# alibaba/EasyParallelLibrary

Measured on AMD Instinct MI355X. Metric: samples_per_sec, higher is better.
Workload: dtype bf16; 1 GPU; model=bert-large, global_batch=128, seq_len=512, parallelism=dp1

## Files before the change

csrc/bindings.hip:

```cpp

#include <hip/hip_runtime.h>
#include <torch/extension.h>
#include <ATen/hip/impl/HIPStreamMasqueradingAsCUDA.h>

#include <cstdint>

namespace epl {
void register_comm(py::module& m);
}

extern "C" {
void epl_fused_adamw(float*, unsigned short*, const void*, bool, float*,
                     float*, int64_t, float, float, float, float, float, int,
                     float, hipStream_t);
void epl_lamb_phase1(const float*, const void*, bool, float*, float*, float*,
                     const int*, float*, float*, int64_t, float, float, float,
                     float, int, float, hipStream_t);
void epl_lamb_phase2(float*, unsigned short*, const float*, const int*,
                     const float*, int64_t, float, hipStream_t);
void epl_layer_norm_fwd(void*, const void*, const void*, void*, const void*,
                        const void*, float*, float*, int64_t, int64_t, float,
                        bool, hipStream_t);
void epl_layer_norm_bwd(void*, float*, float*, const void*, const void*,
                        const void*, const float*, const float*, float*,
                        float*, int64_t, int64_t, int64_t, bool,
                        hipStream_t);
void epl_bias_gelu_fwd(void*, const void*, const void*, int64_t, int64_t,
                       bool, hipStream_t);
void epl_bias_gelu_bwd(void*, float*, const void*, const void*, const void*,
                       float*, int64_t, int64_t, int64_t, bool,
                       hipStream_t);
void epl_ce_rowstats(const void*, const int64_t*, float*, float*, float*,
                     int64_t, int64_t, int64_t, int64_t, bool, hipStream_t);
void epl_ce_backward(void*, const void*, const int64_t*, const float*,
                     const float*, const float*, int64_t, int64_t, int64_t,
                     int64_t, float, bool, hipStream_t);
void epl_scale(void*, int64_t, float, bool, hipStream_t);
void epl_f32_to_bf16(unsigned short*, const float*, int64_t, hipStream_t);
void epl_bf16_to_f32(float*, const unsigned short*, int64_t, hipStream_t);
void epl_sqnorm(const void*, int64_t, float*, bool, hipStream_t);
void epl_colsum(void*, const void*, float*, int64_t, int64_t, int64_t,
                bool, hipStream_t);
void run_mfma_probe(const unsigned short*, const unsigned short*, float*,
                    hipStream_t);
void run_tr_read_probe(short*, short*, int, hipStream_t);
void epl_moe_dispatch_fwd(void*, const void*, const int64_t*,
                          const int64_t*, const int64_t*, int64_t, int64_t,
                          int64_t, hipStream_t);
void epl_moe_dispatch_bwd(void*, const void*, const int64_t*,
                          const int64_t*, const int64_t*, int64_t, int64_t,
                          int64_t, int64_t, hipStream_t);
void epl_moe_combine_fwd(void*, const void*, const float*, const int64_t*,
                         const int64_t*, const int64_t*, int64_t, int64_t,
                         int64_t, int64_t, hipStream_t);
void epl_moe_combine_bwd(void*, float*, const void*, const void*,
                         const float*, const int64_t*, const int64_t*,
                         const int64_t*, int64_t, int64_t, int64_t,
                         hipStream_t);
void epl_attn_fwd(const void*, const void*, const void*, void*, float*,
// ... 107 lines not shown
                     cols, (float)eps, bf16, cur_stream());
}

void layer_norm_bwd(at::Tensor dx, at::Tensor dgamma, at::Tensor dbeta,
                    at::Tensor dy, at::Tensor x, at::Tensor gamma,
                    at::Tensor mean, at::Tensor rstd) {
  const bool bf16 = is_bf16(x);
  const int64_t cols = x.size(-1);
  const int64_t rows = x.numel() / cols;
  TORCH_CHECK(!bf16 || cols % 8 == 0, "bf16 LayerNorm needs cols % 8 == 0");
  TORCH_CHECK((size_t)cols * 2 * sizeof(float) <= 128 * 1024,
              "LayerNorm backward supports cols <= 16384");
  check(dgamma, at::kFloat, "dgamma");
  check(dbeta, at::kFloat, "dbeta");
  float* dgp = nullptr;
  float* dbp = nullptr;
  at::Tensor ws;
  const bool fast = bf16 && cols % 8 == 0 && cols <= 2048;
  int64_t nparts = 0;
  if (fast) {
    const int64_t wave_rows = (rows + 3) / 4;
    nparts = (wave_rows < 1024 ? wave_rows : 1024) * 4;
    ws = at::empty({2, nparts, cols}, dgamma.options());
    dgp = ws.data_ptr<float>();
    dbp = dgp + nparts * cols;
  }
  epl_layer_norm_bwd(dx.data_ptr(), dgamma.data_ptr<float>(),
                     dbeta.data_ptr<float>(), dy.data_ptr(), x.data_ptr(),
                     gamma.data_ptr(), mean.data_ptr<float>(),
                     rstd.data_ptr<float>(), dgp, dbp, nparts, rows, cols,
                     bf16, cur_stream());
}

void bias_gelu_fwd(at::Tensor out, at::Tensor x, at::Tensor bias) {
  const bool bf16 = is_bf16(x);
  const int64_t cols = x.size(-1);
  const int64_t rows = x.numel() / cols;
  TORCH_CHECK(!bf16 || cols % 8 == 0, "bf16 bias_gelu needs cols % 8 == 0");
  epl_bias_gelu_fwd(out.data_ptr(), x.data_ptr(), bias.data_ptr(), rows, cols,
                    bf16, cur_stream());
}

void bias_gelu_bwd(at::Tensor dx, at::Tensor dbias, at::Tensor dy,
                   at::Tensor x, at::Tensor bias) {
  const bool bf16 = is_bf16(x);
  const int64_t cols = x.size(-1);
  const int64_t rows = x.numel() / cols;
  TORCH_CHECK(!bf16 || cols % 8 == 0, "bf16 bias_gelu needs cols % 8 == 0");
  TORCH_CHECK((size_t)cols * sizeof(float) <= 128 * 1024,
              "bias_gelu backward supports cols <= 32768");
  check(dbias, at::kFloat, "dbias");
  float* dbp = nullptr;
  int64_t nwaves = 0;
  at::Tensor ws;
  if (bf16 && cols % 512 == 0) {
    const int64_t segs = cols / 512;
    int64_t per_seg = rows < 1024 ? rows : 1024;
    per_seg = (per_seg + 3) / 4 * 4;
    nwaves = segs * per_seg;
    ws = at::empty({nwaves, 512}, dbias.options());
    dbp = ws.data_ptr<float>();
  }
  epl_bias_gelu_bwd(dx.data_ptr(), dbias.data_ptr<float>(), dy.data_ptr(),
                    x.data_ptr(), bias.data_ptr(), dbp, nwaves, rows, cols,
                    bf16, cur_stream());
}
// ... 220 lines not shown
}

void colsum(at::Tensor dy, at::Tensor db, at::Tensor partial) {
  const bool bf16 = is_bf16(dy);
  TORCH_CHECK(dy.is_cuda() && dy.is_contiguous() && dy.dim() == 2,
              "dy must be a contiguous 2-D device tensor");
  const int64_t rows = dy.size(0), cols = dy.size(1);
  TORCH_CHECK(cols % 8 == 0, "cols must be a multiple of 8");
  TORCH_CHECK(db.numel() == cols && db.scalar_type() == dy.scalar_type());
  const int64_t stripes = partial.numel() / cols;
  TORCH_CHECK(stripes >= 1 && partial.scalar_type() == at::kFloat);
  epl_colsum(db.data_ptr(), dy.data_ptr(), partial.data_ptr<float>(), rows,
             cols, stripes, bf16, cur_stream());
}

void sqnorm(at::Tensor t, at::Tensor out) {
  const bool bf16 = is_bf16(t);
  check(out, at::kFloat, "out");
  epl_sqnorm(t.data_ptr(), t.numel(), out.data_ptr<float>(), bf16,
             cur_stream());
}

}

PYBIND11_MODULE(TORCH_EXTENSION_NAME, m) {
  m.doc() = "MI355X-native parallel library: RCCL comm core + CDNA4 kernels";
  epl::register_comm(m);
  m.def("fused_adamw", &fused_adamw);
  m.def("colsum", &colsum);
  m.def("lamb_phase1", &lamb_phase1);
  m.def("lamb_phase2", &lamb_phase2);
  m.def("layer_norm_fwd", &layer_norm_fwd);
  m.def("layer_norm_bwd", &layer_norm_bwd);
  m.def("bias_gelu_fwd", &bias_gelu_fwd);
  m.def("bias_gelu_bwd", &bias_gelu_bwd);
  m.def("ce_rowstats", &ce_rowstats);
  m.def("ce_backward", &ce_backward);
  m.def("scale_", &scale_);
  m.def("f32_to_bf16", &f32_to_bf16);
  m.def("bf16_to_f32", &bf16_to_f32);
  m.def("sqnorm", &sqnorm);
  m.def("mfma_probe", &mfma_probe);
  m.def("tr_read_probe", &tr_read_probe);
  m.def("moe_dispatch_fwd", &moe_dispatch_fwd);
  m.def("moe_dispatch_bwd", &moe_dispatch_bwd);
  m.def("moe_combine_fwd", &moe_combine_fwd);
  m.def("moe_combine_bwd", &moe_combine_bwd);
  m.def("attn_fwd", &attn_fwd);
  m.def("attn_bwd", &attn_bwd);
}
```

csrc/kernels/kernels.hip:

```cpp

#include <hip/hip_runtime.h>
#include <hip/hip_bf16.h>
#include <cstdint>
#include <cmath>

#define DEV __device__ __forceinline__

namespace {

constexpr int kBlock = 256;
constexpr int kMaxGrid = 4096;

DEV float bf2f(unsigned short u) {
  unsigned int x = (unsigned int)u << 16;
  return __uint_as_float(x);
}

DEV unsigned short f2bf(float f) {
  unsigned int x = __float_as_uint(f);
  unsigned int lsb = (x >> 16) & 1u;
  x += 0x7fffu + lsb;
  return (unsigned short)(x >> 16);
}

// ... 266 lines not shown
          reinterpret_cast<float*>(sum_out)[base + c] = fv;
      }
      sum += fv;
      sumsq += fv * fv;
    }
    sum = block_reduce_sum(sum, lds);
    __syncthreads();
    sumsq = block_reduce_sum(sumsq, lds);
    const float mean = sum / cols;
    const float var = sumsq / cols - mean * mean;
    const float rstd = rsqrtf(var + eps);
    if (threadIdx.x == 0) {
      mean_out[row] = mean;
      rstd_out[row] = rstd;
    }
    const void* nin = HAS_RES ? sum_out : x;
    for (int64_t c = threadIdx.x; c < cols; c += blockDim.x) {
      float fv = BF16 ? bf2f(reinterpret_cast<const T*>(nin)[base + c])
                      : reinterpret_cast<const float*>(nin)[base + c];
      float gv = BF16 ? bf2f(reinterpret_cast<const T*>(gamma)[c])
                      : reinterpret_cast<const float*>(gamma)[c];
      float bv = BF16 ? bf2f(reinterpret_cast<const T*>(beta)[c])
                      : reinterpret_cast<const float*>(beta)[c];
      float y = (fv - mean) * rstd * gv + bv;
      if (BF16)
        reinterpret_cast<T*>(out)[base + c] = f2bf(y);
      else
        reinterpret_cast<float*>(out)[base + c] = y;
    }
    __syncthreads();
  }
}

template <int CHUNKS, bool CACHE>
__global__ __launch_bounds__(256, 2) void layer_norm_bwd_bf16_kernel(
    void* __restrict__ dx, float* __restrict__ dg_part,
    float* __restrict__ db_part, const void* __restrict__ dy,
    const void* __restrict__ x, const void* __restrict__ gamma,
    const float* __restrict__ mean_in, const float* __restrict__ rstd_in,
    int64_t rows, int64_t cols) {
  using T = unsigned short;
  const int lane = threadIdx.x & 63;
  const int wid = threadIdx.x >> 6;
  const int wpb = blockDim.x >> 6;
  float8 gw[CHUNKS], acc_dg[CHUNKS], acc_db[CHUNKS];
#pragma unroll
  for (int k = 0; k < CHUNKS; ++k) {
    const int64_t c = ((int64_t)lane + k * 64) * 8;
#pragma unroll
    for (int j = 0; j < 8; ++j) {
      acc_dg[k].v[j] = 0.f;
      acc_db[k].v[j] = 0.f;
    }
    if (c < cols)
      gw[k] = load_bf16x8(reinterpret_cast<const T*>(gamma) + c);
  }
  for (int64_t row = (int64_t)blockIdx.x * wpb + wid; row < rows;
       row += (int64_t)gridDim.x * wpb) {
    const int64_t base = row * cols;
    const float mean = mean_in[row];
    const float rstd = rstd_in[row];
    float sum_dyg = 0.f, sum_dygx = 0.f;
    float8 c_xhat[CACHE ? CHUNKS : 1], c_dy[CACHE ? CHUNKS : 1];
#pragma unroll
    for (int k = 0; k < CHUNKS; ++k) {
      const int64_t c = ((int64_t)lane + k * 64) * 8;
      if (c >= cols) continue;
      float8 d = load_bf16x8(reinterpret_cast<const T*>(dy) + base + c);
      float8 f = load_bf16x8(reinterpret_cast<const T*>(x) + base + c);
#pragma unroll
      for (int j = 0; j < 8; ++j) {
        const float xhat = (f.v[j] - mean) * rstd;
        const float dyg = d.v[j] * gw[k].v[j];
        if (CACHE) {
          c_xhat[k].v[j] = xhat;
          c_dy[k].v[j] = d.v[j];
        }
        sum_dyg += dyg;
        sum_dygx += dyg * xhat;
      }
    }
#pragma unroll
    for (int off = 32; off > 0; off >>= 1) {
      sum_dyg += __shfl_down(sum_dyg, off, 64);
      sum_dygx += __shfl_down(sum_dygx, off, 64);
    }
    sum_dyg = __shfl(sum_dyg, 0, 64);
    sum_dygx = __shfl(sum_dygx, 0, 64);
    const float inv_cols = 1.f / cols;
#pragma unroll
    for (int k = 0; k < CHUNKS; ++k) {
      const int64_t c = ((int64_t)lane + k * 64) * 8;
      if (c >= cols) continue;
      float8 dv, xh;
      if (CACHE) {
        dv = c_dy[k];
        xh = c_xhat[k];
      } else {
        float8 d = load_bf16x8(reinterpret_cast<const T*>(dy) + base + c);
        float8 f = load_bf16x8(reinterpret_cast<const T*>(x) + base + c);
#pragma unroll
        for (int j = 0; j < 8; ++j) {
          dv.v[j] = d.v[j];
          xh.v[j] = (f.v[j] - mean) * rstd;
        }
      }
      float8 o;
#pragma unroll
      for (int j = 0; j < 8; ++j) {
        const float dyg = dv.v[j] * gw[k].v[j];
        o.v[j] = (dyg - (sum_dyg + xh.v[j] * sum_dygx) * inv_cols) * rstd;
        acc_dg[k].v[j] += dv.v[j] * xh.v[j];
        acc_db[k].v[j] += dv.v[j];
      }
      store_bf16x8(reinterpret_cast<T*>(dx) + base + c, o);
    }
  }
  const int64_t prow = ((int64_t)blockIdx.x * wpb + wid) * cols;
#pragma unroll
  for (int k = 0; k < CHUNKS; ++k) {
    const int64_t c = ((int64_t)lane + k * 64) * 8;
    if (c >= cols) continue;
    store_f32x8(dg_part + prow + c, acc_dg[k]);
    store_f32x8(db_part + prow + c, acc_db[k]);
  }
}

__global__ void ln_bwd_partial_reduce_kernel(
    float* __restrict__ dgamma, float* __restrict__ dbeta,
    const float* __restrict__ dg_part, const float* __restrict__ db_part,
    int64_t nparts, int64_t cols) {
  const int64_t c = (int64_t)blockIdx.x * blockDim.x + threadIdx.x;
  if (c >= cols) return;
  float sg = 0.f, sb = 0.f;
  for (int64_t p = blockIdx.y; p < nparts; p += gridDim.y) {
    sg += dg_part[p * cols + c];
    sb += db_part[p * cols + c];
  }
  atomicAdd(&dgamma[c], sg);
  atomicAdd(&dbeta[c], sb);
}

template <bool BF16>
__global__ void layer_norm_bwd_kernel(
    void* __restrict__ dx, float* __restrict__ dgamma,
    float* __restrict__ dbeta, const void* __restrict__ dy,
    const void* __restrict__ x, const void* __restrict__ gamma,
    const float* __restrict__ mean_in, const float* __restrict__ rstd_in,
    int64_t rows, int64_t cols) {
  extern __shared__ __attribute__((aligned(16))) char smem[];
  float* part_dg = reinterpret_cast<float*>(smem);
  float* part_db = part_dg + cols;
  __shared__ float lds[8];
  using T = unsigned short;
  for (int64_t c = threadIdx.x; c < cols; c += blockDim.x) {
    part_dg[c] = 0.f;
    part_db[c] = 0.f;
  }
  __syncthreads();
  for (int64_t row = blockIdx.x; row < rows; row += gridDim.x) {
    const int64_t base = row * cols;
    const float mean = mean_in[row];
    const float rstd = rstd_in[row];
    float sum_dyg = 0.f, sum_dygx = 0.f;
    for (int64_t c = threadIdx.x; c < cols; c += blockDim.x) {
      const float dv = BF16 ? bf2f(reinterpret_cast<const T*>(dy)[base + c])
                            : reinterpret_cast<const float*>(dy)[base + c];
      const float fv = BF16 ? bf2f(reinterpret_cast<const T*>(x)[base + c])
                            : reinterpret_cast<const float*>(x)[base + c];
      const float gv = BF16 ? bf2f(reinterpret_cast<const T*>(gamma)[c])
                            : reinterpret_cast<const float*>(gamma)[c];
      const float xhat = (fv - mean) * rstd;
      const float dyg = dv * gv;
// ... 18 lines not shown
      const float o = (dv * gv - (sum_dyg + xhat * sum_dygx) * inv_cols) *
                      rstd;
      if (BF16)
        reinterpret_cast<T*>(dx)[base + c] = f2bf(o);
      else
        reinterpret_cast<float*>(dx)[base + c] = o;
    }
    __syncthreads();
  }
  for (int64_t c = threadIdx.x; c < cols; c += blockDim.x) {
    atomicAdd(&dgamma[c], part_dg[c]);
    atomicAdd(&dbeta[c], part_db[c]);
  }
}

DEV float fast_tanh(float u) {
  return 1.f - 2.f / (__expf(2.f * u) + 1.f);
}

DEV float gelu_f(float x) {
  const float k0 = 0.7978845608028654f;
  const float k1 = 0.044715f;
  return 0.5f * x * (1.f + fast_tanh(k0 * (x + k1 * x * x * x)));
}

DEV float gelu_grad_f(float x) {
  const float k0 = 0.7978845608028654f;
  const float k1 = 0.044715f;
  const float t = fast_tanh(k0 * (x + k1 * x * x * x));
  const float dt = (1.f - t * t) * k0 * (1.f + 3.f * k1 * x * x);
  return 0.5f * (1.f + t) + 0.5f * x * dt;
}

template <bool BF16>
__global__ void bias_gelu_fwd_kernel(void* __restrict__ out,
                                     const void* __restrict__ x,
                                     const void* __restrict__ bias,
                                     int64_t rows, int64_t cols) {
  using T = unsigned short;
  const int64_t n = rows * cols;
  if (BF16) {
    const int64_t nvec = n / 8;
    for (int64_t i = blockIdx.x * blockDim.x + threadIdx.x; i < nvec;
         i += (int64_t)gridDim.x * blockDim.x) {
      const int64_t base = i * 8;
      float8 f = load_bf16x8(reinterpret_cast<const T*>(x) + base);
      float8 b = load_bf16x8(reinterpret_cast<const T*>(bias) +
                             (base % cols));
      float8 o;
#pragma unroll
      for (int k = 0; k < 8; ++k) o.v[k] = gelu_f(f.v[k] + b.v[k]);
      store_bf16x8(reinterpret_cast<T*>(out) + base, o);
    }
  } else {
    for (int64_t i = blockIdx.x * blockDim.x + threadIdx.x; i < n;
         i += (int64_t)gridDim.x * blockDim.x) {
      const float xv = reinterpret_cast<const float*>(x)[i] +
                       reinterpret_cast<const float*>(bias)[i % cols];
      reinterpret_cast<float*>(out)[i] = gelu_f(xv);
    }
  }
}

__global__ void bias_gelu_bwd_bf16_kernel(
    void* __restrict__ dx, float* __restrict__ db_part,
    const void* __restrict__ dy, const void* __restrict__ x,
    const void* __restrict__ bias, int64_t rows, int64_t cols) {
  using T = unsigned short;
  const int lane = threadIdx.x & 63;
  const int wid = threadIdx.x >> 6;
  const int wpb = blockDim.x >> 6;
  const int64_t segs = cols / 512;
  const int64_t total = rows * segs;
  float8 acc;
#pragma unroll
  for (int j = 0; j < 8; ++j) acc.v[j] = 0.f;
  const int64_t wave_id = (int64_t)blockIdx.x * wpb + wid;
  const int64_t nwaves = (int64_t)gridDim.x * wpb;
  const int64_t myseg = wave_id % segs;
  const int64_t c0 = myseg * 512 + (int64_t)lane * 8;
  float8 bw = load_bf16x8(reinterpret_cast<const T*>(bias) + c0);
  for (int64_t row = wave_id / segs; row < rows; row += nwaves / segs) {
    const int64_t base = row * cols + c0;
    float8 d = load_bf16x8(reinterpret_cast<const T*>(dy) + base);
    float8 f = load_bf16x8(reinterpret_cast<const T*>(x) + base);
    float8 o;
#pragma unroll
    for (int j = 0; j < 8; ++j) {
      const float g = d.v[j] * gelu_grad_f(f.v[j] + bw.v[j]);
      o.v[j] = g;
      acc.v[j] += g;
    }
    store_bf16x8(reinterpret_cast<T*>(dx) + base, o);
  }
  store_f32x8(db_part + wave_id * 512 + (int64_t)lane * 8, acc);
}

__global__ void bias_gelu_db_reduce_kernel(
    float* __restrict__ dbias, const float* __restrict__ db_part,
    int64_t nwaves, int64_t segs) {
  const int64_t c = (int64_t)blockIdx.x * blockDim.x + threadIdx.x;
  if (c >= segs * 512) return;
  const int64_t seg = c / 512;
  const int64_t off = c % 512;
  float sum = 0.f;
  for (int64_t p = seg + blockIdx.y * segs; p < nwaves;
       p += (int64_t)gridDim.y * segs) {
    sum += db_part[p * 512 + off];
  }
  atomicAdd(&dbias[c], sum);
}

template <bool BF16>
__global__ void bias_gelu_bwd_kernel(void* __restrict__ dx,
                                     float* __restrict__ dbias,
                                     const void* __restrict__ dy,
                                     const void* __restrict__ x,
                                     const void* __restrict__ bias,
                                     int64_t rows, int64_t cols) {
  extern __shared__ __attribute__((aligned(16))) char smem[];
  float* part_db = reinterpret_cast<float*>(smem);
  using T = unsigned short;
  for (int64_t c = threadIdx.x; c < cols; c += blockDim.x) part_db[c] = 0.f;
  __syncthreads();
  for (int64_t row = blockIdx.x; row < rows; row += gridDim.x) {
    const int64_t base = row * cols;
// ... 224 lines not shown
  if (c >= cols) return;
  const int64_t per = (rows + stripes - 1) / stripes;
  const int64_t r0 = (int64_t)blockIdx.y * per;
  const int64_t r1 = r0 + per < rows ? r0 + per : rows;
  float8 acc = {};
  for (int64_t r = r0; r < r1; ++r) {
    if (BF16) {
      const float8 v =
          load_bf16x8(reinterpret_cast<const unsigned short*>(dy) +
                      r * cols + c);
#pragma unroll
      for (int k = 0; k < 8; ++k) acc.v[k] += v.v[k];
    } else {
      const float* p = reinterpret_cast<const float*>(dy) + r * cols + c;
#pragma unroll
      for (int k = 0; k < 8; ++k) acc.v[k] += p[k];
    }
  }
  store_f32x8(partial + (int64_t)blockIdx.y * cols + c, acc);
}

template <bool BF16>
__global__ void colsum_reduce_kernel(void* __restrict__ db,
                                     const float* __restrict__ partial,
                                     int64_t stripes, int64_t cols) {
  const int64_t c = (int64_t)blockIdx.x * blockDim.x + threadIdx.x;
  if (c >= cols) return;
  float s = 0.f;
  for (int64_t p = 0; p < stripes; ++p) s += partial[p * cols + c];
  if (BF16)
    reinterpret_cast<unsigned short*>(db)[c] = f2bf(s);
  else
    reinterpret_cast<float*>(db)[c] = s;
}

extern "C" {

void epl_fused_adamw(float* master, unsigned short* param_bf16,
                     const void* grad, bool grad_bf16, float* m, float* v,
                     int64_t n, float lr, float beta1, float beta2, float eps,
                     float weight_decay, int step, float inv_scale,
                     hipStream_t stream) {
  const float inv_bias1 = 1.f / (1.f - powf(beta1, (float)step));
  const float inv_bias2 = 1.f / (1.f - powf(beta2, (float)step));
  const int grid = grid_for((n + 7) / 8);
  if (grad_bf16) {
    if (param_bf16)
      hipLaunchKernelGGL((fused_adamw_kernel<true, true>), dim3(grid),
                         dim3(kBlock), 0, stream, master, param_bf16, grad, m,
                         v, n, lr, beta1, beta2, eps, weight_decay, inv_bias1,
                         inv_bias2, inv_scale);
    else
      hipLaunchKernelGGL((fused_adamw_kernel<true, false>), dim3(grid),
                         dim3(kBlock), 0, stream, master, param_bf16, grad, m,
                         v, n, lr, beta1, beta2, eps, weight_decay, inv_bias1,
                         inv_bias2, inv_scale);
  } else {
    if (param_bf16)
      hipLaunchKernelGGL((fused_adamw_kernel<false, true>), dim3(grid),
                         dim3(kBlock), 0, stream, master, param_bf16, grad, m,
                         v, n, lr, beta1, beta2, eps, weight_decay, inv_bias1,
                         inv_bias2, inv_scale);
    else
      hipLaunchKernelGGL((fused_adamw_kernel<false, false>), dim3(grid),
                         dim3(kBlock), 0, stream, master, param_bf16, grad, m,
                         v, n, lr, beta1, beta2, eps, weight_decay, inv_bias1,
// ... 53 lines not shown
    } else {
      if (two)
        hipLaunchKernelGGL((layer_norm_fwd_bf16_kernel<false, 2>), dim3(grid),
                           dim3(block), 0, stream, out, x, res, sum_out,
                           gamma, beta, mean, rstd, rows, cols, eps);
      else
        hipLaunchKernelGGL((layer_norm_fwd_bf16_kernel<false, 1>), dim3(grid),
                           dim3(block), 0, stream, out, x, res, sum_out,
                           gamma, beta, mean, rstd, rows, cols, eps);
    }
    return;
  }
  if (bf16) {
    if (has_res)
      hipLaunchKernelGGL((layer_norm_fwd_kernel<true, true>), dim3(grid),
                         dim3(kBlock), 0, stream, out, x, res, sum_out,
                         gamma, beta, mean, rstd, rows, cols, eps);
    else
      hipLaunchKernelGGL((layer_norm_fwd_kernel<true, false>), dim3(grid),
                         dim3(kBlock), 0, stream, out, x, res, sum_out,
                         gamma, beta, mean, rstd, rows, cols, eps);
  } else {
    if (has_res)
      hipLaunchKernelGGL((layer_norm_fwd_kernel<false, true>), dim3(grid),
                         dim3(kBlock), 0, stream, out, x, res, sum_out,
                         gamma, beta, mean, rstd, rows, cols, eps);
    else
      hipLaunchKernelGGL((layer_norm_fwd_kernel<false, false>), dim3(grid),
                         dim3(kBlock), 0, stream, out, x, res, sum_out,
                         gamma, beta, mean, rstd, rows, cols, eps);
  }
}

void epl_layer_norm_bwd(void* dx, float* dgamma, float* dbeta, const void* dy,
                        const void* x, const void* gamma, const float* mean,
                        const float* rstd, float* dg_part, float* db_part,
                        int64_t nparts, int64_t rows, int64_t cols,
                        bool bf16, hipStream_t stream) {
  if (bf16 && cols % 8 == 0 && cols <= 2048 && dg_part != nullptr) {
    const int64_t wave_rows = (rows + 3) / 4;
    const int grid = (int)(wave_rows < 1024 ? wave_rows : 1024);
    if (cols <= 512)
      hipLaunchKernelGGL((layer_norm_bwd_bf16_kernel<1, true>), dim3(grid),
                         dim3(256), 0, stream, dx, dg_part, db_part, dy, x,
                         gamma, mean, rstd, rows, cols);
    else if (cols <= 1024)
      hipLaunchKernelGGL((layer_norm_bwd_bf16_kernel<2, true>), dim3(grid),
                         dim3(256), 0, stream, dx, dg_part, db_part, dy, x,
                         gamma, mean, rstd, rows, cols);
    else
      hipLaunchKernelGGL((layer_norm_bwd_bf16_kernel<4, false>),
                         dim3(grid), dim3(256), 0, stream, dx, dg_part,
                         db_part, dy, x, gamma, mean, rstd, rows, cols);
    hipLaunchKernelGGL(ln_bwd_partial_reduce_kernel,
                       dim3((unsigned)((cols + 255) / 256), 64), dim3(256),
                       0, stream, dgamma, dbeta, dg_part, db_part,
                       (int64_t)grid * 4, cols);
    return;
  }
  int grid = (int)(rows < 1024 ? rows : 1024);
  const size_t lds_bytes = (size_t)cols * 2 * sizeof(float);
  if (bf16)
    hipLaunchKernelGGL((layer_norm_bwd_kernel<true>), dim3(grid),
                       dim3(kBlock), lds_bytes, stream, dx, dgamma, dbeta,
                       dy, x, gamma, mean, rstd, rows, cols);
  else
    hipLaunchKernelGGL((layer_norm_bwd_kernel<false>), dim3(grid),
                       dim3(kBlock), lds_bytes, stream, dx, dgamma, dbeta,
                       dy, x, gamma, mean, rstd, rows, cols);
}

void epl_bias_gelu_fwd(void* out, const void* x, const void* bias,
                       int64_t rows, int64_t cols, bool bf16,
                       hipStream_t stream) {
  const int grid = grid_for((rows * cols + 7) / 8);
  if (bf16)
    hipLaunchKernelGGL(bias_gelu_fwd_kernel<true>, dim3(grid), dim3(kBlock), 0,
                       stream, out, x, bias, rows, cols);
  else
    hipLaunchKernelGGL(bias_gelu_fwd_kernel<false>, dim3(grid), dim3(kBlock),
                       0, stream, out, x, bias, rows, cols);
}

void epl_bias_gelu_bwd(void* dx, float* dbias, const void* dy, const void* x,
                       const void* bias, float* db_part, int64_t nwaves,
                       int64_t rows, int64_t cols, bool bf16,
                       hipStream_t stream) {
  if (bf16 && cols % 512 == 0 && db_part != nullptr) {
    const int grid = (int)(nwaves / 4);
    hipLaunchKernelGGL(bias_gelu_bwd_bf16_kernel, dim3(grid), dim3(256), 0,
                       stream, dx, db_part, dy, x, bias, rows, cols);
    const int64_t segs = cols / 512;
    hipLaunchKernelGGL(bias_gelu_db_reduce_kernel,
                       dim3((unsigned)((cols + 255) / 256), 32), dim3(256),
                       0, stream, dbias, db_part, nwaves, segs);
    return;
  }
  int grid = (int)(rows < 1024 ? rows : 1024);
  const size_t lds_bytes = (size_t)cols * sizeof(float);
  if (bf16)
    hipLaunchKernelGGL(bias_gelu_bwd_kernel<true>, dim3(grid), dim3(kBlock),
                       lds_bytes, stream, dx, dbias, dy, x, bias, rows,
                       cols);
  else
    hipLaunchKernelGGL(bias_gelu_bwd_kernel<false>, dim3(grid), dim3(kBlock),
                       lds_bytes, stream, dx, dbias, dy, x, bias, rows,
                       cols);
}

void epl_ce_rowstats(const void* logits, const int64_t* targets,
                     float* row_max, float* row_sumexp, float* target_logit,
                     int64_t rows, int64_t cols, int64_t vocab_begin,
// ... 89 lines not shown
```

easyparallellibrary_amd/models/transformer.py:

```python

import os

import torch
import torch.nn as nn
import torch.nn.functional as F

_NATIVE_ATTN = os.environ.get("EPL_NATIVE_ATTENTION", "auto")

from easyparallellibrary_amd.ops.bias_gelu import FusedBiasGelu
from easyparallellibrary_amd.ops.bias_linear import FusedBiasLinear
from easyparallellibrary_amd.ops.layer_norm import FusedLayerNorm

_FBG = os.environ.get("EPL_FUSED_BIAS_GRAD", "0") == "1"
_Linear = FusedBiasLinear if _FBG else nn.Linear

_QKV_SPLIT = os.environ.get("EPL_QKV_SPLIT", "1") == "1"


class _QKVSplit(torch.autograd.Function):

    @staticmethod
    def forward(ctx, qkv):
        q = qkv[:, :, 0].transpose(1, 2)
        k = qkv[:, :, 1].transpose(1, 2)
        v = qkv[:, :, 2].transpose(1, 2)
        return q, k, v

    @staticmethod
    def backward(ctx, dq, dk, dv):
        b, nh, s, d = dq.shape
        dqkv = torch.empty((b, s, 3, nh, d), dtype=dq.dtype,
                           device=dq.device)
        dqkv[:, :, 0].copy_(dq.transpose(1, 2))
        dqkv[:, :, 1].copy_(dk.transpose(1, 2))
        dqkv[:, :, 2].copy_(dv.transpose(1, 2))
        return dqkv


class SelfAttention(nn.Module):
    def __init__(self, hidden, num_heads, causal=False, dropout=0.0):
        super().__init__()
        assert hidden % num_heads == 0
        self.hidden = hidden
        self.num_heads = num_heads
        self.head_dim = hidden // num_heads
        self.causal = causal
        self.qkv = _Linear(hidden, 3 * hidden)
        self.proj = _Linear(hidden, hidden)
        self.dropout = dropout

    def forward(self, x):
        from easyparallellibrary_amd.ops.attention import (
            flash_attention, qkv_flash_attention, qkv_native_ok)
        b, s, h = x.shape
        qkv = self.qkv(x).reshape(b, s, 3, self.num_heads, self.head_dim)
        native_here = _NATIVE_ATTN in ("1", "auto")
        p = self.dropout if self.training else 0.0
        if native_here and qkv_native_ok(qkv):
            o = qkv_flash_attention(qkv, causal=self.causal, dropout_p=p)
            o = o.transpose(1, 2).reshape(b, s, h)
            return self.proj(o)
        if _QKV_SPLIT:
            q, k, v = _QKVSplit.apply(qkv)
        else:
            q, k, v = qkv.unbind(dim=2)
            q = q.transpose(1, 2)
            k = k.transpose(1, 2)
            v = v.transpose(1, 2)
        o = flash_attention(q, k, v, causal=self.causal,
                            allow_native=native_here, dropout_p=p)
        o = o.transpose(1, 2).reshape(b, s, h)
        return self.proj(o)


class MLP(nn.Module):

    def __init__(self, hidden, ffn_hidden):
        super().__init__()
        self.fc1 = nn.Linear(hidden, ffn_hidden, bias=False)
        self.act = FusedBiasGelu(ffn_hidden)
        self.fc2 = _Linear(ffn_hidden, hidden)

    def forward(self, x):
        return self.fc2(self.act(self.fc1(x)))


class Block(nn.Module):

    def __init__(self, hidden, num_heads, ffn_hidden, causal=False,
                 pre_ln=False, dropout=0.0):
        super().__init__()
        self.pre_ln = pre_ln
        self.ln1 = FusedLayerNorm(hidden)
        self.attn = SelfAttention(hidden, num_heads, causal=causal,
                                  dropout=dropout)
        self.ln2 = FusedLayerNorm(hidden)
        self.mlp = MLP(hidden, ffn_hidden)

    def forward(self, x):
        if self.pre_ln:
            a = self.attn(self.ln1(x))
            y, s = self.ln2.forward_with_sum(a, x)
            return s + self.mlp(y)
        x = self.ln1(self.attn(x), residual=x)
        x = self.ln2(self.mlp(x), residual=x)
        return x


class Embeddings(nn.Module):
    def __init__(self, vocab_size, hidden, max_positions, use_ln=True):
        super().__init__()
        self.tok = nn.Embedding(vocab_size, hidden)
        self.pos = nn.Embedding(max_positions, hidden)
        self.ln = FusedLayerNorm(hidden) if use_ln else None
        nn.init.normal_(self.tok.weight, std=0.02)
        nn.init.normal_(self.pos.weight, std=0.02)

    def forward(self, ids):
        s = ids.shape[1]
        pos = torch.arange(s, device=ids.device)
        x = self.tok(ids) + self.pos(pos)[None, :, :]
        if self.ln is not None:
            x = self.ln(x)
        return x


class LMHead(nn.Module):

    def __init__(self, hidden, vocab_size, use_ln=True):
        super().__init__()
        self.ln = FusedLayerNorm(hidden) if use_ln else None
        self.proj = nn.Linear(hidden, vocab_size, bias=False)
        nn.init.normal_(self.proj.weight, std=0.02)

    def forward(self, x):
        if self.ln is not None:
            x = self.ln(x)
        return self.proj(x)
# ... 10 lines not shown
```

easyparallellibrary_amd/ops/layer_norm.py:

```python

import torch
import torch.nn as nn

from easyparallellibrary_amd.ops.dispatch import native_ext, use_native


def _native_ok(x):
    return (use_native(x) and x.dtype in (torch.bfloat16, torch.float32)
            and x.shape[-1] % 8 == 0)


class _FusedLayerNorm(torch.autograd.Function):

    @staticmethod
    def forward(ctx, x, residual, gamma, beta, eps):
        x = x.contiguous()
        cols = x.shape[-1]
        rows = x.numel() // cols
        has_res = residual is not None
        if has_res:
            residual = residual.contiguous().to(x.dtype)
        ctx.param_dtype = gamma.dtype
        gamma = gamma.contiguous().to(x.dtype)
        beta = beta.contiguous().to(x.dtype)
        if _native_ok(x):
            mean = torch.empty(rows, dtype=torch.float32, device=x.device)
            rstd = torch.empty(rows, dtype=torch.float32, device=x.device)
            out = torch.empty_like(x)
            s = torch.empty_like(x) if has_res else None
            native_ext().layer_norm_fwd(out, x, residual, s, gamma,
                                        beta, mean, rstd, eps)
            norm_in = s if has_res else x
        else:
            norm_in = (x + residual) if has_res else x
            xf = norm_in.float().reshape(rows, cols)
            mu = xf.mean(dim=1)
            var = xf.var(dim=1, unbiased=False)
            rstd = (var + eps).rsqrt()
            mean = mu
            xhat = (xf - mu[:, None]) * rstd[:, None]
            out = (xhat * gamma.float() + beta.float()).to(x.dtype)
            out = out.reshape(x.shape)
            s = norm_in if has_res else None
        ctx.save_for_backward(norm_in, gamma, mean, rstd)
        ctx.has_res = has_res
        if has_res:
            return out, s
        return out

    @staticmethod
    def backward(ctx, dy, *rest):
        norm_in, gamma, mean, rstd = ctx.saved_tensors
        ds = rest[0] if (ctx.has_res and rest) else None
        dy = dy.contiguous()
        cols = norm_in.shape[-1]
        rows = norm_in.numel() // cols
        if _native_ok(norm_in):
            dx = torch.empty_like(norm_in)
            dgamma = torch.zeros(cols, dtype=torch.float32,
                                 device=norm_in.device)
            dbeta = torch.zeros(cols, dtype=torch.float32,
                                device=norm_in.device)
            native_ext().layer_norm_bwd(dx, dgamma, dbeta, dy, norm_in,
                                        gamma.contiguous(), mean, rstd)
        else:
            xf = norm_in.float().reshape(rows, cols)
            dyf = dy.float().reshape(rows, cols)
            xhat = (xf - mean[:, None]) * rstd[:, None]
            dyg = dyf * gamma.float()
            c1 = dyg.mean(dim=1, keepdim=True)
            c2 = (dyg * xhat).mean(dim=1, keepdim=True)
            dx = ((dyg - c1 - xhat * c2) * rstd[:, None]).to(norm_in.dtype)
            dx = dx.reshape(norm_in.shape)
            dgamma = (dyf * xhat).sum(dim=0)
            dbeta = dyf.sum(dim=0)
        if ds is not None:
            dx = dx + ds
        if ctx.has_res:
            return (dx, dx, dgamma.to(ctx.param_dtype),
                    dbeta.to(ctx.param_dtype), None)
        return (dx, None, dgamma.to(ctx.param_dtype),
                dbeta.to(ctx.param_dtype), None)


class FusedLayerNorm(nn.Module):
    def __init__(self, hidden, eps=1e-5):
        super().__init__()
        self.weight = nn.Parameter(torch.ones(hidden))
        self.bias = nn.Parameter(torch.zeros(hidden))
        self.eps = eps

    def forward(self, x, residual=None):
        if residual is None:
            return _FusedLayerNorm.apply(x, None, self.weight, self.bias,
                                         self.eps)
        out, _ = _FusedLayerNorm.apply(x, residual, self.weight, self.bias,
                                       self.eps)
        return out

    def forward_with_sum(self, x, residual):
        return _FusedLayerNorm.apply(x, residual, self.weight, self.bias,
                                     self.eps)
```

Measured before the change: 686.9 samples/s.

## Fuse residual-grad add and linear bias-grad colsum into LayerNorm backward kernel

```diff
diff --git a/csrc/bindings.hip b/csrc/bindings.hip
--- a/csrc/bindings.hip
+++ b/csrc/bindings.hip
@@ -25,6 +25,11 @@
                         const void*, const float*, const float*, float*,
                         float*, int64_t, int64_t, int64_t, bool,
                         hipStream_t);
+void epl_layer_norm_bwd_fused(void*, float*, float*, float*, const void*,
+                              const void*, const void*, const void*,
+                              const float*, const float*, float*, float*,
+                              float*, int64_t, int64_t, int64_t, bool,
+                              hipStream_t);
 void epl_bias_gelu_fwd(void*, const void*, const void*, int64_t, int64_t,
                        bool, hipStream_t);
 void epl_bias_gelu_bwd(void*, float*, const void*, const void*, const void*,
@@ -198,6 +203,59 @@
                      bf16, cur_stream());
 }
 
+void layer_norm_bwd_fused(at::Tensor dx, at::Tensor dgamma, at::Tensor dbeta,
+                          at::Tensor dy, at::Tensor x, at::Tensor gamma,
+                          at::Tensor mean, at::Tensor rstd,
+                          c10::optional<at::Tensor> dadd,
+                          c10::optional<at::Tensor> colsum_out) {
+  const bool bf16 = is_bf16(x);
+  const int64_t cols = x.size(-1);
+  const int64_t rows = x.numel() / cols;
+  TORCH_CHECK(!bf16 || cols % 8 == 0, "bf16 LayerNorm needs cols % 8 == 0");
+  TORCH_CHECK((size_t)cols * 2 * sizeof(float) <= 128 * 1024,
+              "LayerNorm backward supports cols <= 16384");
+  check(dgamma, at::kFloat, "dgamma");
+  check(dbeta, at::kFloat, "dbeta");
+  TORCH_CHECK(dx.numel() == x.numel() && dy.numel() == x.numel());
+  TORCH_CHECK(dgamma.numel() == cols && dbeta.numel() == cols);
+  const bool fast = bf16 && cols % 8 == 0 && cols <= 2048;
+  const bool fused = dadd.has_value() || colsum_out.has_value();
+  TORCH_CHECK(fast || !fused,
+              "layer_norm_bwd_fused: dadd/colsum_out need the bf16 fast "
+              "path (cols % 8 == 0, cols <= 2048)");
+  const void* dadd_p = nullptr;
+  float* cs_out = nullptr;
+  if (dadd.has_value()) {
+    check(*dadd, x.scalar_type(), "dadd");
+    TORCH_CHECK(dadd->numel() == x.numel(), "dadd shape mismatch");
+    dadd_p = dadd->data_ptr();
+  }
+  if (colsum_out.has_value()) {
+    check(*colsum_out, at::kFloat, "colsum_out");
+    TORCH_CHECK(colsum_out->numel() == cols, "colsum_out shape mismatch");
+    cs_out = colsum_out->data_ptr<float>();
+  }
+  float* dgp = nullptr;
+  float* dbp = nullptr;
+  float* csp = nullptr;
+  at::Tensor ws;
+  int64_t nparts = 0;
+  if (fast) {
+    const int64_t wave_rows = (rows + 3) / 4;
+    nparts = (wave_rows < 1024 ? wave_rows : 1024) * 4;
+    ws = at::empty({cs_out ? 3 : 2, nparts, cols}, dgamma.options());
+    dgp = ws.data_ptr<float>();
+    dbp = dgp + nparts * cols;
+    if (cs_out) csp = dbp + nparts * cols;
+  }
+  epl_layer_norm_bwd_fused(dx.data_ptr(), dgamma.data_ptr<float>(),
+                           dbeta.data_ptr<float>(), cs_out, dy.data_ptr(),
+                           x.data_ptr(), gamma.data_ptr(), dadd_p,
+                           mean.data_ptr<float>(), rstd.data_ptr<float>(),
+                           dgp, dbp, csp, nparts, rows, cols, bf16,
+                           cur_stream());
+}
+
 void bias_gelu_fwd(at::Tensor out, at::Tensor x, at::Tensor bias) {
   const bool bf16 = is_bf16(x);
   const int64_t cols = x.size(-1);
@@ -484,6 +542,10 @@
   m.def("lamb_phase2", &lamb_phase2);
   m.def("layer_norm_fwd", &layer_norm_fwd);
   m.def("layer_norm_bwd", &layer_norm_bwd);
+  m.def("layer_norm_bwd_fused", &layer_norm_bwd_fused, py::arg("dx"),
+        py::arg("dgamma"), py::arg("dbeta"), py::arg("dy"), py::arg("x"),
+        py::arg("gamma"), py::arg("mean"), py::arg("rstd"),
+        py::arg("dadd") = py::none(), py::arg("colsum_out") = py::none());
   m.def("bias_gelu_fwd", &bias_gelu_fwd);
   m.def("bias_gelu_bwd", &bias_gelu_bwd);
   m.def("ce_rowstats", &ce_rowstats);
diff --git a/csrc/kernels/kernels.hip b/csrc/kernels/kernels.hip
--- a/csrc/kernels/kernels.hip
+++ b/csrc/kernels/kernels.hip
@@ -322,18 +322,44 @@
   }
 }
 
-template <int CHUNKS, bool CACHE>
-__global__ __launch_bounds__(256, 2) void layer_norm_bwd_bf16_kernel(
+template <int CHUNKS, bool CACHE, bool DADD, bool COLSUM>
+__global__ __launch_bounds__(256, CHUNKS == 1 ? 5 : 3) void
+layer_norm_bwd_bf16_kernel(
     void* __restrict__ dx, float* __restrict__ dg_part,
-    float* __restrict__ db_part, const void* __restrict__ dy,
-    const void* __restrict__ x, const void* __restrict__ gamma,
+    float* __restrict__ db_part, float* __restrict__ cs_part,
+    const void* __restrict__ dy, const void* __restrict__ x,
+    const void* __restrict__ gamma, const void* __restrict__ dadd,
     const float* __restrict__ mean_in, const float* __restrict__ rstd_in,
     int64_t rows, int64_t cols) {
   using T = unsigned short;
   const int lane = threadIdx.x & 63;
   const int wid = threadIdx.x >> 6;
   const int wpb = blockDim.x >> 6;
-  float8 gw[CHUNKS], acc_dg[CHUNKS], acc_db[CHUNKS];
+  constexpr bool FUSED = DADD || COLSUM;
+  constexpr bool G_LDS = FUSED && CHUNKS == 4;
+  constexpr bool G_PK = FUSED && CHUNKS == 1;
+  constexpr bool G_F32 = !G_LDS && !G_PK;
+  __shared__ __attribute__((aligned(16))) T g_lds[G_LDS ? CHUNKS * 512 : 8];
+  float8 gw[G_F32 ? CHUNKS : 1], acc_dg[CHUNKS], acc_db[CHUNKS];
+  uint4 gpk[G_PK ? CHUNKS : 1];
+  float8 acc_cs[COLSUM ? CHUNKS : 1];
+  if (G_LDS) {
+    for (int64_t c = (int64_t)threadIdx.x * 8; c < cols;
+         c += (int64_t)blockDim.x * 8)
+      *reinterpret_cast<uint4*>(g_lds + c) =
+          *reinterpret_cast<const uint4*>(reinterpret_cast<const T*>(gamma) +
+                                          c);
+    __syncthreads();
+  }
+  auto gamma_at = [&](int k, int64_t c) -> float8 {
+    if (G_LDS) return load_bf16x8(g_lds + c);
+    if (G_PK) {
+      asm volatile("" : "+v"(gpk[k].x), "+v"(gpk[k].y), "+v"(gpk[k].z),
+                   "+v"(gpk[k].w));
+      return load_bf16x8(reinterpret_cast<const T*>(&gpk[k]));
+    }
+    return gw[k];
+  };
 #pragma unroll
   for (int k = 0; k < CHUNKS; ++k) {
     const int64_t c = ((int64_t)lane + k * 64) * 8;
@@ -341,9 +367,15 @@
     for (int j = 0; j < 8; ++j) {
       acc_dg[k].v[j] = 0.f;
       acc_db[k].v[j] = 0.f;
-    }
-    if (c < cols)
-      gw[k] = load_bf16x8(reinterpret_cast<const T*>(gamma) + c);
+      if (COLSUM) acc_cs[k].v[j] = 0.f;
+    }
+    if (c < cols) {
+      if (G_F32)
+        gw[k] = load_bf16x8(reinterpret_cast<const T*>(gamma) + c);
+      if (G_PK)
+        gpk[k] = *reinterpret_cast<const uint4*>(
+            reinterpret_cast<const T*>(gamma) + c);
+    }
   }
   for (int64_t row = (int64_t)blockIdx.x * wpb + wid; row < rows;
        row += (int64_t)gridDim.x * wpb) {
@@ -358,10 +390,11 @@
       if (c >= cols) continue;
       float8 d = load_bf16x8(reinterpret_cast<const T*>(dy) + base + c);
       float8 f = load_bf16x8(reinterpret_cast<const T*>(x) + base + c);
+      const float8 g = gamma_at(k, c);
 #pragma unroll
       for (int j = 0; j < 8; ++j) {
         const float xhat = (f.v[j] - mean) * rstd;
-        const float dyg = d.v[j] * gw[k].v[j];
+        const float dyg = d.v[j] * g.v[j];
         if (CACHE) {
           c_xhat[k].v[j] = xhat;
           c_dy[k].v[j] = d.v[j];
@@ -395,13 +428,24 @@
           xh.v[j] = (f.v[j] - mean) * rstd;
         }
       }
+      const float8 g = gamma_at(k, c);
       float8 o;
 #pragma unroll
       for (int j = 0; j < 8; ++j) {
-        const float dyg = dv.v[j] * gw[k].v[j];
+        const float dyg = dv.v[j] * g.v[j];
         o.v[j] = (dyg - (sum_dyg + xh.v[j] * sum_dygx) * inv_cols) * rstd;
         acc_dg[k].v[j] += dv.v[j] * xh.v[j];
         acc_db[k].v[j] += dv.v[j];
+      }
+      if (DADD) {
+        const float8 a =
+            load_bf16x8(reinterpret_cast<const T*>(dadd) + base + c);
+#pragma unroll
+        for (int j = 0; j < 8; ++j) o.v[j] += a.v[j];
+      }
+      if (COLSUM) {
+#pragma unroll
+        for (int j = 0; j < 8; ++j) acc_cs[k].v[j] += o.v[j];
       }
       store_bf16x8(reinterpret_cast<T*>(dx) + base + c, o);
     }
@@ -413,22 +457,27 @@
     if (c >= cols) continue;
     store_f32x8(dg_part + prow + c, acc_dg[k]);
     store_f32x8(db_part + prow + c, acc_db[k]);
-  }
-}
-
+    if (COLSUM) store_f32x8(cs_part + prow + c, acc_cs[k]);
+  }
+}
+
+template <bool COLSUM>
 __global__ void ln_bwd_partial_reduce_kernel(
     float* __restrict__ dgamma, float* __restrict__ dbeta,
-    const float* __restrict__ dg_part, const float* __restrict__ db_part,
+    float* __restrict__ colsum, const float* __restrict__ dg_part,
+    const float* __restrict__ db_part, const float* __restrict__ cs_part,
     int64_t nparts, int64_t cols) {
   const int64_t c = (int64_t)blockIdx.x * blockDim.x + threadIdx.x;
   if (c >= cols) return;
-  float sg = 0.f, sb = 0.f;
+  float sg = 0.f, sb = 0.f, sc = 0.f;
   for (int64_t p = blockIdx.y; p < nparts; p += gridDim.y) {
     sg += dg_part[p * cols + c];
     sb += db_part[p * cols + c];
+    if (COLSUM) sc += cs_part[p * cols + c];
   }
   atomicAdd(&dgamma[c], sg);
   atomicAdd(&dbeta[c], sb);
+  if (COLSUM) atomicAdd(&colsum[c], sc);
 }
 
 template <bool BF16>
@@ -513,6 +562,38 @@
   return 0.5f * (1.f + t) + 0.5f * x * dt;
 }
 
+DEV float gelu_sigmoid(float x) {
+  constexpr float c0 = (float)(-2.0 * 0.7978845608028654 *
+                               1.4426950408889634);
+  constexpr float c1 = (float)(-2.0 * 0.7978845608028654 *
+                               1.4426950408889634 * 0.044715);
+  const float e = __builtin_amdgcn_exp2f(x * (c0 + c1 * x * x));
+  return __builtin_amdgcn_rcpf(1.f + e);
+}
+
+DEV float gelu_lean(float x) { return x * gelu_sigmoid(x); }
+
+DEV float gelu_grad_lean(float x) {
+  constexpr float d0 = (float)(2.0 * 0.7978845608028654);
+  constexpr float d1 = (float)(6.0 * 0.7978845608028654 * 0.044715);
+  const float s = gelu_sigmoid(x);
+  return s + x * s * (1.f - s) * (d0 + d1 * x * x);
+}
+
+using f32x2 = __attribute__((ext_vector_type(2))) float;
+using bf16v2 = __attribute__((ext_vector_type(2))) __bf16;
+
+DEV unsigned int cvt_pk_bf16(float a, float b) {
+  f32x2 f = {a, b};
+  return __builtin_bit_cast(unsigned int, __builtin_convertvector(f, bf16v2));
+}
+
+DEV void store_bf16x8_pk(unsigned short* p, const float8& f) {
+  *reinterpret_cast<uint4*>(p) =
+      make_uint4(cvt_pk_bf16(f.v[0], f.v[1]), cvt_pk_bf16(f.v[2], f.v[3]),
+                 cvt_pk_bf16(f.v[4], f.v[5]), cvt_pk_bf16(f.v[6], f.v[7]));
+}
+
 template <bool BF16>
 __global__ void bias_gelu_fwd_kernel(void* __restrict__ out,
                                      const void* __restrict__ x,
@@ -521,17 +602,20 @@
   using T = unsigned short;
   const int64_t n = rows * cols;
   if (BF16) {
-    const int64_t nvec = n / 8;
-    for (int64_t i = blockIdx.x * blockDim.x + threadIdx.x; i < nvec;
-         i += (int64_t)gridDim.x * blockDim.x) {
-      const int64_t base = i * 8;
+    const unsigned vpr = (unsigned)(cols / 8);
+    const unsigned g = blockIdx.x * blockDim.x + threadIdx.x;
+    const unsigned rpp = (gridDim.x * blockDim.x) / vpr;
+    const unsigned r0 = g / vpr;
+    if (r0 >= rpp) return;
+    const int64_t c = (int64_t)(g - r0 * vpr) * 8;
+    const float8 b = load_bf16x8(reinterpret_cast<const T*>(bias) + c);
+    for (int64_t row = r0; row < rows; row += rpp) {
+      const int64_t base = row * cols + c;
       float8 f = load_bf16x8(reinterpret_cast<const T*>(x) + base);
-      float8 b = load_bf16x8(reinterpret_cast<const T*>(bias) +
-                             (base % cols));
       float8 o;
 #pragma unroll
-      for (int k = 0; k < 8; ++k) o.v[k] = gelu_f(f.v[k] + b.v[k]);
-      store_bf16x8(reinterpret_cast<T*>(out) + base, o);
+      for (int k = 0; k < 8; ++k) o.v[k] = gelu_lean(f.v[k] + b.v[k]);
+      store_bf16x8_pk(reinterpret_cast<T*>(out) + base, o);
     }
   } else {
     for (int64_t i = blockIdx.x * blockDim.x + threadIdx.x; i < n;
@@ -568,11 +652,11 @@
     float8 o;
 #pragma unroll
     for (int j = 0; j < 8; ++j) {
-      const float g = d.v[j] * gelu_grad_f(f.v[j] + bw.v[j]);
+      const float g = d.v[j] * gelu_grad_lean(f.v[j] + bw.v[j]);
       o.v[j] = g;
       acc.v[j] += g;
     }
-    store_bf16x8(reinterpret_cast<T*>(dx) + base, o);
+    store_bf16x8_pk(reinterpret_cast<T*>(dx) + base, o);
   }
   store_f32x8(db_part + wave_id * 512 + (int64_t)lane * 8, acc);
 }
@@ -863,6 +947,37 @@
     reinterpret_cast<unsigned short*>(db)[c] = f2bf(s);
   else
     reinterpret_cast<float*>(db)[c] = s;
+}
+
+template <bool DADD, bool COLSUM>
+static void ln_bwd_fast_launch(void* dx, float* dgamma, float* dbeta,
+                               float* colsum, const void* dy, const void* x,
+                               const void* gamma, const void* dadd,
+                               const float* mean, const float* rstd,
+                               float* dg_part, float* db_part,
+                               float* cs_part, int64_t rows, int64_t cols,
+                               hipStream_t stream) {
+  const int64_t wave_rows = (rows + 3) / 4;
+  const int grid = (int)(wave_rows < 1024 ? wave_rows : 1024);
+  if (cols <= 512)
+    hipLaunchKernelGGL((layer_norm_bwd_bf16_kernel<1, true, DADD, COLSUM>),
+                       dim3(grid), dim3(256), 0, stream, dx, dg_part,
+                       db_part, cs_part, dy, x, gamma, dadd, mean, rstd,
+                       rows, cols);
+  else if (cols <= 1024)
+    hipLaunchKernelGGL((layer_norm_bwd_bf16_kernel<2, true, DADD, COLSUM>),
+                       dim3(grid), dim3(256), 0, stream, dx, dg_part,
+                       db_part, cs_part, dy, x, gamma, dadd, mean, rstd,
+                       rows, cols);
+  else
+    hipLaunchKernelGGL((layer_norm_bwd_bf16_kernel<4, false, DADD, COLSUM>),
+                       dim3(grid), dim3(256), 0, stream, dx, dg_part,
+                       db_part, cs_part, dy, x, gamma, dadd, mean, rstd,
+                       rows, cols);
+  hipLaunchKernelGGL(ln_bwd_partial_reduce_kernel<COLSUM>,
+                     dim3((unsigned)((cols + 255) / 256), 64), dim3(256), 0,
+                     stream, dgamma, dbeta, colsum, dg_part, db_part,
+                     cs_part, (int64_t)grid * 4, cols);
 }
 
 extern "C" {
@@ -982,30 +1097,35 @@
   }
 }
 
-void epl_layer_norm_bwd(void* dx, float* dgamma, float* dbeta, const void* dy,
-                        const void* x, const void* gamma, const float* mean,
-                        const float* rstd, float* dg_part, float* db_part,
-                        int64_t nparts, int64_t rows, int64_t cols,
-                        bool bf16, hipStream_t stream) {
+void epl_layer_norm_bwd_fused(void* dx, float* dgamma, float* dbeta,
+                              float* colsum, const void* dy, const void* x,
+                              const void* gamma, const void* dadd,
+                              const float* mean, const float* rstd,
+                              float* dg_part, float* db_part,
+                              float* cs_part, int64_t nparts, int64_t rows,
+                              int64_t cols, bool bf16, hipStream_t stream) {
   if (bf16 && cols % 8 == 0 && cols <= 2048 && dg_part != nullptr) {
-    const int64_t wave_rows = (rows + 3) / 4;
-    const int grid = (int)(wave_rows < 1024 ? wave_rows : 1024);
-    if (cols <= 512)
-      hipLaunchKernelGGL((layer_norm_bwd_bf16_kernel<1, true>), dim3(grid),
-                         dim3(256), 0, stream, dx, dg_part, db_part, dy, x,
-                         gamma, mean, rstd, rows, cols);
-    else if (cols <= 1024)
-      hipLaunchKernelGGL((layer_norm_bwd_bf16_kernel<2, true>), dim3(grid),
-                         dim3(256), 0, stream, dx, dg_part, db_part, dy, x,
-                         gamma, mean, rstd, rows, cols);
-    else
-      hipLaunchKernelGGL((layer_norm_bwd_bf16_kernel<4, false>),
-                         dim3(grid), dim3(256), 0, stream, dx, dg_part,
-                         db_part, dy, x, gamma, mean, rstd, rows, cols);
-    hipLaunchKernelGGL(ln_bwd_partial_reduce_kernel,
-                       dim3((unsigned)((cols + 255) / 256), 64), dim3(256),
-                       0, stream, dgamma, dbeta, dg_part, db_part,
-                       (int64_t)grid * 4, cols);
+    const bool has_cs = colsum != nullptr && cs_part != nullptr;
+    if (dadd != nullptr) {
+      if (has_cs)
+        ln_bwd_fast_launch<true, true>(dx, dgamma, dbeta, colsum, dy, x,
+                                       gamma, dadd, mean, rstd, dg_part,
+                                       db_part, cs_part, rows, cols, stream);
+      else
+        ln_bwd_fast_launch<true, false>(dx, dgamma, dbeta, colsum, dy, x,
+                                        gamma, dadd, mean, rstd, dg_part,
+                                        db_part, cs_part, rows, cols, stream);
+    } else {
+      if (has_cs)
+        ln_bwd_fast_launch<false, true>(dx, dgamma, dbeta, colsum, dy, x,
+                                        gamma, dadd, mean, rstd, dg_part,
+                                        db_part, cs_part, rows, cols, stream);
+      else
+        ln_bwd_fast_launch<false, false>(dx, dgamma, dbeta, colsum, dy, x,
+                                         gamma, dadd, mean, rstd, dg_part,
+                                         db_part, cs_part, rows, cols,
+                                         stream);
+    }
     return;
   }
   int grid = (int)(rows < 1024 ? rows : 1024);
@@ -1020,14 +1140,26 @@
                        dy, x, gamma, mean, rstd, rows, cols);
 }
 
+void epl_layer_norm_bwd(void* dx, float* dgamma, float* dbeta, const void* dy,
+                        const void* x, const void* gamma, const float* mean,
+                        const float* rstd, float* dg_part, float* db_part,
+                        int64_t nparts, int64_t rows, int64_t cols,
+                        bool bf16, hipStream_t stream) {
+  epl_layer_norm_bwd_fused(dx, dgamma, dbeta, nullptr, dy, x, gamma, nullptr,
+                           mean, rstd, dg_part, db_part, nullptr, nparts,
+                           rows, cols, bf16, stream);
+}
+
 void epl_bias_gelu_fwd(void* out, const void* x, const void* bias,
                        int64_t rows, int64_t cols, bool bf16,
                        hipStream_t stream) {
-  const int grid = grid_for((rows * cols + 7) / 8);
-  if (bf16)
+  int grid = grid_for((rows * cols + 7) / 8);
+  if (bf16) {
+    const int min_grid = (int)((cols / 8 + kBlock - 1) / kBlock);
+    if (grid < min_grid) grid = min_grid;
     hipLaunchKernelGGL(bias_gelu_fwd_kernel<true>, dim3(grid), dim3(kBlock), 0,
                        stream, out, x, bias, rows, cols);
-  else
+  } else
     hipLaunchKernelGGL(bias_gelu_fwd_kernel<false>, dim3(grid), dim3(kBlock),
                        0, stream, out, x, bias, rows, cols);
 }
diff --git a/easyparallellibrary_amd/models/transformer.py b/easyparallellibrary_amd/models/transformer.py
--- a/easyparallellibrary_amd/models/transformer.py
+++ b/easyparallellibrary_amd/models/transformer.py
@@ -9,7 +9,8 @@
 
 from easyparallellibrary_amd.ops.bias_gelu import FusedBiasGelu
 from easyparallellibrary_amd.ops.bias_linear import FusedBiasLinear
-from easyparallellibrary_amd.ops.layer_norm import FusedLayerNorm
+from easyparallellibrary_amd.ops.layer_norm import (FusedLayerNorm,
+                                                    linear_for_ln)
 
 _FBG = os.environ.get("EPL_FUSED_BIAS_GRAD", "0") == "1"
 _Linear = FusedBiasLinear if _FBG else nn.Linear
@@ -49,7 +50,13 @@
         self.proj = _Linear(hidden, hidden)
         self.dropout = dropout
 
-    def forward(self, x):
+    def forward(self, x, bias_grad_to_ln=False):
+        o = self._attend(x)
+        if bias_grad_to_ln:
+            return linear_for_ln(self.proj, o)
+        return self.proj(o)
+
+    def _attend(self, x):
         from easyparallellibrary_amd.ops.attention import (
             flash_attention, qkv_flash_attention, qkv_native_ok)
         b, s, h = x.shape
@@ -58,8 +65,7 @@
         p = self.dropout if self.training else 0.0
         if native_here and qkv_native_ok(qkv):
             o = qkv_flash_attention(qkv, causal=self.causal, dropout_p=p)
-            o = o.transpose(1, 2).reshape(b, s, h)
-            return self.proj(o)
+            return o.transpose(1, 2).reshape(b, s, h)
         if _QKV_SPLIT:
             q, k, v = _QKVSplit.apply(qkv)
         else:
@@ -69,8 +75,7 @@
             v = v.transpose(1, 2)
         o = flash_attention(q, k, v, causal=self.causal,
                             allow_native=native_here, dropout_p=p)
-        o = o.transpose(1, 2).reshape(b, s, h)
-        return self.proj(o)
+        return o.transpose(1, 2).reshape(b, s, h)
 
 
 class MLP(nn.Module):
@@ -81,8 +86,11 @@
         self.act = FusedBiasGelu(ffn_hidden)
         self.fc2 = _Linear(ffn_hidden, hidden)
 
-    def forward(self, x):
-        return self.fc2(self.act(self.fc1(x)))
+    def forward(self, x, bias_grad_to_ln=False):
+        h = self.act(self.fc1(x))
+        if bias_grad_to_ln:
+            return linear_for_ln(self.fc2, h)
+        return self.fc2(h)
 
 
 class Block(nn.Module):
@@ -97,13 +105,21 @@
         self.ln2 = FusedLayerNorm(hidden)
         self.mlp = MLP(hidden, ffn_hidden)
 
+    @staticmethod
+    def _into_ln(mod, cls, x):
+        if type(mod) is cls:
+            return mod(x, bias_grad_to_ln=True)
+        return mod(x), None
+
     def forward(self, x):
         if self.pre_ln:
-            a = self.attn(self.ln1(x))
-            y, s = self.ln2.forward_with_sum(a, x)
+            a, pb = self._into_ln(self.attn, SelfAttention, self.ln1(x))
+            y, s = self.ln2.forward_with_sum(a, x, lin_bias=pb)
             return s + self.mlp(y)
-        x = self.ln1(self.attn(x), residual=x)
-        x = self.ln2(self.mlp(x), residual=x)
+        a, pb = self._into_ln(self.attn, SelfAttention, x)
+        x = self.ln1(a, residual=x, lin_bias=pb)
+        m, fb = self._into_ln(self.mlp, MLP, x)
+        x = self.ln2(m, residual=x, lin_bias=fb)
         return x
 
 
diff --git a/easyparallellibrary_amd/ops/layer_norm.py b/easyparallellibrary_amd/ops/layer_norm.py
--- a/easyparallellibrary_amd/ops/layer_norm.py
+++ b/easyparallellibrary_amd/ops/layer_norm.py
@@ -1,8 +1,14 @@
+
+import os
 
 import torch
 import torch.nn as nn
+import torch.nn.functional as F
 
 from easyparallellibrary_amd.ops.dispatch import native_ext, use_native
+
+
+_LN_BWD_FUSE = os.environ.get("EPL_LN_BWD_FUSE", "1") == "1"
 
 
 def _native_ok(x):
@@ -10,10 +16,37 @@
             and x.shape[-1] % 8 == 0)
 
 
+def _bwd_fast_ok(x):
+    return (_native_ok(x) and x.dtype == torch.bfloat16
+            and x.shape[-1] <= 2048)
+
+
+def layer_norm_bwd_fused(dy, x, gamma, mean, rstd, dadd=None,
+                         want_colsum=False):
+    cols = x.shape[-1]
+    dx = torch.empty_like(x)
+    dgamma = torch.zeros(cols, dtype=torch.float32, device=x.device)
+    dbeta = torch.zeros(cols, dtype=torch.float32, device=x.device)
+    if _bwd_fast_ok(x):
+        colsum = (torch.zeros(cols, dtype=torch.float32, device=x.device)
+                  if want_colsum else None)
+        if dadd is not None:
+            dadd = dadd.contiguous().to(x.dtype)
+        native_ext().layer_norm_bwd_fused(dx, dgamma, dbeta, dy, x, gamma,
+                                          mean, rstd, dadd, colsum)
+        return dx, dgamma, dbeta, colsum
+    native_ext().layer_norm_bwd(dx, dgamma, dbeta, dy, x, gamma, mean, rstd)
+    if dadd is not None:
+        dx = dx + dadd
+    colsum = (dx.reshape(-1, cols).sum(dim=0, dtype=torch.float32)
+              if want_colsum else None)
+    return dx, dgamma, dbeta, colsum
+
+
 class _FusedLayerNorm(torch.autograd.Function):
 
     @staticmethod
-    def forward(ctx, x, residual, gamma, beta, eps):
+    def forward(ctx, x, residual, gamma, beta, eps, lin_bias=None):
         x = x.contiguous()
         cols = x.shape[-1]
         rows = x.numel() // cols
@@ -44,6 +77,10 @@
             s = norm_in if has_res else None
         ctx.save_for_backward(norm_in, gamma, mean, rstd)
         ctx.has_res = has_res
+        ctx.bias_dtype = lin_bias.dtype if lin_bias is not None else None
+        ctx.fuse = _LN_BWD_FUSE
+        if ctx.fuse:
+            ctx.set_materialize_grads(False)
         if has_res:
             return out, s
         return out
@@ -52,17 +89,22 @@
     def backward(ctx, dy, *rest):
         norm_in, gamma, mean, rstd = ctx.saved_tensors
         ds = rest[0] if (ctx.has_res and rest) else None
-        dy = dy.contiguous()
+        ds_late = None
+        if not ctx.fuse:
+            ds, ds_late = None, ds
+        want_db = ctx.bias_dtype is not None and ctx.needs_input_grad[5]
         cols = norm_in.shape[-1]
         rows = norm_in.numel() // cols
-        if _native_ok(norm_in):
-            dx = torch.empty_like(norm_in)
-            dgamma = torch.zeros(cols, dtype=torch.float32,
-                                 device=norm_in.device)
-            dbeta = torch.zeros(cols, dtype=torch.float32,
-                                device=norm_in.device)
-            native_ext().layer_norm_bwd(dx, dgamma, dbeta, dy, norm_in,
-                                        gamma.contiguous(), mean, rstd)
+        dgamma = dbeta = colsum = None
+        if dy is None:
+            dx = ds
+            if dx is not None and want_db:
+                colsum = dx.reshape(rows, cols).sum(dim=0,
+                                                    dtype=torch.float32)
+        elif _native_ok(norm_in):
+            dx, dgamma, dbeta, colsum = layer_norm_bwd_fused(
+                dy.contiguous(), norm_in, gamma.contiguous(), mean, rstd,
+                dadd=ds, want_colsum=want_db)
         else:
             xf = norm_in.float().reshape(rows, cols)
             dyf = dy.float().reshape(rows, cols)
@@ -70,17 +112,21 @@
             dyg = dyf * gamma.float()
             c1 = dyg.mean(dim=1, keepdim=True)
             c2 = (dyg * xhat).mean(dim=1, keepdim=True)
-            dx = ((dyg - c1 - xhat * c2) * rstd[:, None]).to(norm_in.dtype)
-            dx = dx.reshape(norm_in.shape)
+            dxf = (dyg - c1 - xhat * c2) * rstd[:, None]
+            if ds is not None:
+                dxf = dxf + ds.float().reshape(rows, cols)
+            if want_db:
+                colsum = dxf.sum(dim=0)
+            dx = dxf.to(norm_in.dtype).reshape(norm_in.shape)
             dgamma = (dyf * xhat).sum(dim=0)
             dbeta = dyf.sum(dim=0)
-        if ds is not None:
-            dx = dx + ds
-        if ctx.has_res:
-            return (dx, dx, dgamma.to(ctx.param_dtype),
-                    dbeta.to(ctx.param_dtype), None)
-        return (dx, None, dgamma.to(ctx.param_dtype),
-                dbeta.to(ctx.param_dtype), None)
+        if dgamma is not None:
+            dgamma = dgamma.to(ctx.param_dtype)
+            dbeta = dbeta.to(ctx.param_dtype)
+        if ds_late is not None:
+            dx = dx + ds_late
+        dbias = colsum.to(ctx.bias_dtype) if colsum is not None else None
+        return (dx, dx if ctx.has_res else None, dgamma, dbeta, None, dbias)
 
 
 class FusedLayerNorm(nn.Module):
@@ -90,14 +136,21 @@
         self.bias = nn.Parameter(torch.zeros(hidden))
         self.eps = eps
 
-    def forward(self, x, residual=None):
+    def forward(self, x, residual=None, lin_bias=None):
         if residual is None:
             return _FusedLayerNorm.apply(x, None, self.weight, self.bias,
-                                         self.eps)
+                                         self.eps, lin_bias)
         out, _ = _FusedLayerNorm.apply(x, residual, self.weight, self.bias,
-                                       self.eps)
+                                       self.eps, lin_bias)
         return out
 
-    def forward_with_sum(self, x, residual):
+    def forward_with_sum(self, x, residual, lin_bias=None):
         return _FusedLayerNorm.apply(x, residual, self.weight, self.bias,
-                                     self.eps)
+                                     self.eps, lin_bias)
+
+
+def linear_for_ln(lin, x):
+    if (_LN_BWD_FUSE and type(lin) is nn.Linear and lin.bias is not None
+            and lin.bias.requires_grad and torch.is_grad_enabled()):
+        return F.linear(x, lin.weight, lin.bias.detach()), lin.bias
+    return lin(x), None
```

Result: faster. 718.6 samples/s, median of 6 (+4.6%).
